# apple/ml-fastvlm

Hardware: AMD Instinct MI355X
Metric: images/sec FastViTHD encode_images @1024x1024 bf16 (higher is better)
Workload: dtype bf16; 1 GPU; BASELINE.json configs[1]: FastViTHD encoder + mlp2x_gelu projector (H=896), batch=32/GPU synthetic 1024x1024 bf16 images in [0,1), seeded synthetic weights, single GPU; global_batch=32, image_size=1024, parallelism=dp1, hip_graph=False, attention_operands=bf16, ffn_precision=auto (calibrated on the benchmark batch), range guard on

## Files before the change

ml_fastvlm_amd/csrc/ffn_fused.hip:

```cpp
#include "fvhd_common.h"
#include <stdlib.h>

typedef float f32x16 __attribute__((ext_vector_type(16)));

template <int C> __host__ __device__ __forceinline__ int w1_off(int row, int slot)
{
    if constexpr (C == 384) return row * 768 + ((slot ^ (row & 15)) << 4);
    else if constexpr (C == 192) return row * 384 + ((slot ^ ((row >> 1) & 7)) << 4);
    else return row * 192 + ((slot ^ ((row >> 2) & 3)) << 4);
}

__host__ __device__ __forceinline__ int w2_off(int row, int slot)
{
    return row * 64 + ((slot ^ ((row >> 2) & 3)) << 4);
}

struct GeluSt { f32x2 x, xc, u, q; };
#define FFN_PK(c) (f32x2{c, c})
#ifndef FVHD_FFN_GELU_DEG
#define FVHD_FFN_GELU_DEG 5
#endif
template <int H> FVHD_DEV void gelu_half(GeluSt& g, f32x2 x, f32x2& out)
{
#if FVHD_FFN_GELU_DEG == 7
    if constexpr (H == 0) {
        g.x = x;
        g.xc = f32x2{__builtin_amdgcn_fmed3f(x[0], -FVHD_GELU_CLAMP, FVHD_GELU_CLAMP), __builtin_amdgcn_fmed3f(x[1], -FVHD_GELU_CLAMP, FVHD_GELU_CLAMP)};
    } else if constexpr (H == 1) {
        g.u = g.xc * g.xc;
        g.q = __builtin_elementwise_fma(FFN_PK(FVHD_GELU_C7), g.u, FFN_PK(FVHD_GELU_C6));
    } else if constexpr (H == 2) {
        g.q = __builtin_elementwise_fma(g.q, g.u, FFN_PK(FVHD_GELU_C5));
        g.q = __builtin_elementwise_fma(g.q, g.u, FFN_PK(FVHD_GELU_C4));
    } else if constexpr (H == 3) {
        g.q = __builtin_elementwise_fma(g.q, g.u, FFN_PK(FVHD_GELU_C3));
        g.q = __builtin_elementwise_fma(g.q, g.u, FFN_PK(FVHD_GELU_C2));
    } else if constexpr (H == 4) {
        g.q = __builtin_elementwise_fma(g.q, g.u, FFN_PK(FVHD_GELU_C1));
        g.q = __builtin_elementwise_fma(g.q, g.u, FFN_PK(FVHD_GELU_C0));
    } else {
        out = g.x * __builtin_elementwise_fma(g.xc, g.q, FFN_PK(0.5f));
    }
#else
    if constexpr (H == 0) {
        g.x = x;
        g.xc = f32x2{__builtin_amdgcn_fmed3f(x[0], -FVHD_GELU5_CLAMP, FVHD_GELU5_CLAMP), __builtin_amdgcn_fmed3f(x[1], -FVHD_GELU5_CLAMP, FVHD_GELU5_CLAMP)};
    } else if constexpr (H == 1) {
        g.u = g.xc * g.xc;
        g.q = __builtin_elementwise_fma(FFN_PK(FVHD_GELU5_C5), g.u, FFN_PK(FVHD_GELU5_C4));
    } else if constexpr (H == 2) {
        g.q = __builtin_elementwise_fma(g.q, g.u, FFN_PK(FVHD_GELU5_C3));
    } else if constexpr (H == 3) {
        g.q = __builtin_elementwise_fma(g.q, g.u, FFN_PK(FVHD_GELU5_C2));
    } else if constexpr (H == 4) {
        g.q = __builtin_elementwise_fma(g.q, g.u, FFN_PK(FVHD_GELU5_C1));
        g.q = __builtin_elementwise_fma(g.q, g.u, FFN_PK(FVHD_GELU5_C0));
    } else {
        out = g.x * __builtin_elementwise_fma(g.xc, g.q, FFN_PK(0.5f));
    }
#endif
}

#ifndef FVHD_FFN_CIO384
#define FVHD_FFN_CIO384 1
#endif
#ifndef FVHD_FFN_PAIRWAIT
#define FVHD_FFN_PAIRWAIT 1
#endif
#ifndef FVHD_FFN_DMARUN
#define FVHD_FFN_DMARUN 1
#endif
#ifndef FVHD_FFN_F16
#define FVHD_FFN_F16 2
#endif
template <int C> __host__ __device__ constexpr bool ffn_f16() { return FVHD_FFN_F16 == 2 || (FVHD_FFN_F16 == 1 && C <= 192); }
typedef _Float16 f16x2 __attribute__((ext_vector_type(2)));
typedef _Float16 f16x8 __attribute__((ext_vector_type(8)));
struct GeluSt16 { f16x2 x, u, q; };
#define FFN_H2(bits) (__builtin_bit_cast(f16x2, (unsigned)(bits) * 0x10001u))
template <int K> FVHD_DEV void gelu16_stage(GeluSt16& g, f32x2 x, f16x2& out)
{
    if constexpr (K == 0) g.x = __builtin_bit_cast(f16x2, __builtin_amdgcn_cvt_pkrtz(x[0], x[1]));
    else if constexpr (K == 1) g.u = g.x * g.x;
    else if constexpr (K == 2) g.u = __builtin_elementwise_min(g.u, FFN_H2(0x3a20));
    else if constexpr (K == 3) g.q = __builtin_elementwise_fma(FFN_H2(0xc1b0), g.u, FFN_H2(0x4878));
    else if constexpr (K == 4) g.q = __builtin_elementwise_fma(g.q, g.u, FFN_H2(0xc9e5));
    else if constexpr (K == 5) g.q = __builtin_elementwise_fma(g.q, g.u, FFN_H2(0x485a));
    else if constexpr (K == 6) g.q = __builtin_elementwise_fma(g.q, g.u, FFN_H2(0xc41f));
    else if constexpr (K == 7) g.q = __builtin_elementwise_fma(g.q, g.u, FFN_H2(0x3e5f));
    else if constexpr (K == 8) asm("v_pk_fma_f16 %0, %1, %2, %3 clamp" : "=v"(g.q) : "v"(g.x), "v"(g.q), "v"(FFN_H2(0x3800)));
    else out = g.x * g.q;
}
template <int K = 0> FVHD_DEV void gelu16_dispatch(int k, GeluSt16& g, f32x2 x, f16x2& out)
{
    if constexpr (K < 10) {
        if (k == K) gelu16_stage<K>(g, x, out);
        else gelu16_dispatch<K + 1>(k, g, x, out);
    }
}

#ifdef FVHD_FFN_ABL_NOWAIT
FVHD_DEV void ffn_wait_dma() {}
#else
FVHD_DEV void ffn_wait_dma() { asm volatile("s_waitcnt vmcnt(0)" ::: "memory"); }
#endif

template <int C, int NB, int WAVES, bool DO_A, bool DO_B, bool DO_C, bool DO_DMA, int VAR, int PF, bool F16 = ffn_f16<C>(), bool BPRE = (C == 96 || F16)>
FVHD_DEV void ffn_iter(const bf16x8 (&afr)[NB][C / 16], f32x16 (&o)[NB][C / 32], f32x16 (&s_out)[NB], const f32x16 (&s_in)[NB],
                       bf16x8 (&p_out)[NB][2], const bf16x8 (&p_in)[NB][2], const char* const (&w1p)[C / 48],
                       const char* const (&w2p)[2], const int ring, const float* b1_cur, const float* b1_prev, int half,
                       const char* dma_src1, unsigned dma_dst1, bool dma1, const char* dma_src2, unsigned dma_dst2, bool dma2, int uwave)
{
    constexpr int KS = C / 16, NF = 2 * KS, NM = NF * NB;
    constexpr int NA = C / 48, CHB = 64 * C, NG = CHB / 1024;
    constexpr int UPS = 96 * NB / NM;
    constexpr int DW = WAVES, TP = 2 * NG, NPW = (TP + DW - 1) / DW;
    static_assert(TP % DW == 0, "every wave issues the same number of pieces");
    constexpr bool PIN = !(VAR & 16);
    constexpr int DSTRIDE = (VAR & 32) ? 1 : ((NM / 2) / NPW > 0 ? (NM / 2) / NPW : 1);
#define FFN_LD_W1(ks) (*(const bf16x8*)(w1p[(ks) % NA] + ring * CHB + ((ks) / NA) * NA * 32))
#define FFN_LD_W2(f) (*(const bf16x8*)(w2p[(f) & 1] + ring * CHB + ((f) >> 1) * 2048))
#define FFN_LD(f) (((f) & 1) ? FFN_LD_W2((f) >> 1) : FFN_LD_W1((f) >> 1))
#define FFN_LD_ON(f) (((f) & 1) ? DO_C : DO_A)
    bf16x8 wf[NF];
    f32x4 bv[4];
    GeluSt gs[NB][8];
    f32x2 gout[NB][8];
    GeluSt16 gs16[NB][8];
    f16x2 gout16[NB][8];
    if constexpr (DO_A && BPRE) {
#pragma unroll
        for (int q = 0; q < 4; ++q) bv[q] = *(const f32x4*)(b1_cur + 8 * q + 4 * half);
    }
    if constexpr (DO_B && !BPRE) bv[0] = *(const f32x4*)(b1_prev + 4 * half);
    constexpr bool PAIRW = FVHD_FFN_PAIRWAIT && PIN && F16 && BPRE && NB == 1 && DO_A && DO_B && DO_C && !(VAR & (4 | 8));
    constexpr int PFE = PAIRW ? 4 : PF;
#pragma unroll
    for (int f = 0; f < PFE; ++f)
        if (FFN_LD_ON(f)) wf[f] = FFN_LD(f);
    if constexpr (PIN) __builtin_amdgcn_sched_barrier(0);
#pragma unroll
    for (int m = 0; m < NM; ++m) {
        const int f = m / NB, nb = m % NB;
        if constexpr (PAIRW) {
            if ((f & 1) == 0) {
                if (f + 2 < NF) __builtin_amdgcn_s_waitcnt(0xc27f);
                else __builtin_amdgcn_s_waitcnt(0xc07f);
            }
        }
        if ((f & 1) == 0) {
            if constexpr (DO_A) {
                const int ks = f >> 1;
                if constexpr (VAR & 8) asm volatile("" ::"v"(wf[f]));
                else if (ks == 0) {
                    f32x16 z;
#pragma unroll
                    for (int r = 0; r < 16; ++r) z[r] = BPRE ? bv[r >> 2][r & 3] : 0.0f;
                    s_out[nb] = __builtin_amdgcn_mfma_f32_32x32x16_bf16(wf[f], afr[nb][ks], z, 0, 0, 0);
                } else s_out[nb] = __builtin_amdgcn_mfma_f32_32x32x16_bf16(wf[f], afr[nb][ks], s_out[nb], 0, 0, 0);
            }
        } else {
            if constexpr (DO_C) {
                const int g = f >> 1;
                if constexpr (VAR & 4) asm volatile("" ::"v"(wf[f]), "v"(p_in[nb][g & 1]));
                else if constexpr (F16)
                    o[nb][g >> 1] = __builtin_amdgcn_mfma_f32_32x32x16_f16(__builtin_bit_cast(f16x8, wf[f]), __builtin_bit_cast(f16x8, p_in[nb][g & 1]), o[nb][g >> 1], 0, 0, 0);
                else o[nb][g >> 1] = __builtin_amdgcn_mfma_f32_32x32x16_bf16(wf[f], p_in[nb][g & 1], o[nb][g >> 1], 0, 0, 0);
            }
        }
        if constexpr (PIN) __builtin_amdgcn_sched_barrier(0);
        if constexpr (PAIRW) {
            if ((f & 1) == 0) {
                if (f + 4 < NF) wf[f + 4] = FFN_LD(f + 4);
                if (f + 5 < NF) wf[f + 5] = FFN_LD(f + 5);
            }
        } else if (nb == 0 && f + PF < NF && FFN_LD_ON(f + PF)) wf[f + PF] = FFN_LD(f + PF);
        if constexpr (DO_DMA) {
#if FVHD_FFN_DMARUN
            constexpr int PPW = TP / DW, RUN = PPW % 4 == 0 ? 4 : PPW % 3 == 0 ? 3 : PPW, NRUN = PPW / RUN, RSTRIDE = (NM / 2) / NRUN > 0 ? (NM / 2) / NRUN : 1;
            static_assert(TP % DW == 0 && PPW % RUN == 0 && RUN <= 4 && DW % 2 == 0 && NG % PPW == 0, "a wave's pieces lie in one matrix");
            if (m % RSTRIDE == 0 && m / RSTRIDE < NRUN) {
                const int second = uwave >= DW / 2;
                const unsigned pc0 = (unsigned)((uwave % (DW / 2)) * PPW + (m / RSTRIDE) * RUN) * 1024u;
                const char* sb = (second ? dma_src2 : dma_src1) + pc0;
                const unsigned dst = (second ? dma_dst2 : dma_dst1) + pc0;
                if (second ? dma2 : dma1) glds16_run<RUN>(sb, (threadIdx.x & 63) * 16u, dst);
            }
#else
            if (m % DSTRIDE == 0 && m / DSTRIDE < NPW) {
                const int flat = (m / DSTRIDE) * DW + uwave;
                const int lane16 = (threadIdx.x & 63) * 16;
                const bool second = flat >= NG;
                const int pc = second ? flat - NG : flat;
                const char* src = (second ? dma_src2 : dma_src1) + pc * 1024 + lane16;
                const unsigned dst = (second ? dma_dst2 : dma_dst1) + (unsigned)pc * 1024u;
                if (second ? dma2 : dma1) glds16(src, dst);
            }
#endif
        }
        if constexpr (DO_B) {
            if constexpr (!BPRE) {
#pragma unroll
                for (int q = 1; q < 4; ++q)
                    if (m == ((24 * q * NB) / UPS >= 2 ? (24 * q * NB) / UPS - 2 : 0)) bv[q] = *(const f32x4*)(b1_prev + 8 * q + 4 * half);
            }
            if constexpr (F16) {
                constexpr int NGRP = NM / 12;
                static_assert(NGRP * UPS == 8 * NB && NGRP * 10 <= NM, "ten stages of every pair group fit into the iteration's slots");
                if (m / 10 < NGRP) {
                    const int k = m % 10;
#pragma unroll
                    for (int i = 0; i < UPS; ++i) {
                        const int pr = (m / 10) * UPS + i, gb = pr % NB, r = 2 * (pr / NB);
                        const f32x2 sv = {s_in[gb][r], s_in[gb][r + 1]};
                        if constexpr (VAR & 2) {
                            if (k == 9) gout16[gb][r >> 1] = __builtin_bit_cast(f16x2, __builtin_amdgcn_cvt_pkrtz(sv[0], sv[1]));
                        } else gelu16_dispatch(k, gs16[gb][r >> 1], sv, gout16[gb][r >> 1]);
                        if (k == 9) {
                            f16x8 pt = __builtin_bit_cast(f16x8, p_out[gb][r >> 3]);
                            pt[r & 7] = gout16[gb][r >> 1][0];
                            pt[(r & 7) + 1] = gout16[gb][r >> 1][1];
                            p_out[gb][r >> 3] = __builtin_bit_cast(bf16x8, pt);
                        }
                    }
                }
            } else
#pragma unroll
            for (int u = m * UPS / 2; u < (m + 1) * UPS / 2; ++u) {
                const int gb = u % NB, jh = u / NB, h = jh % 6, r = 2 * (jh / 6);
                f32x2 sv = {s_in[gb][r], s_in[gb][r + 1]};
                if (!BPRE && (h == 0 || ((VAR & (2 | 64)) && h == 5))) sv += f32x2{bv[r >> 2][r & 3], bv[r >> 2][(r & 3) + 1]};
                if (VAR & 2) {
                    if (h == 5) gout[gb][r >> 1] = sv;
                } else {
                    if constexpr (VAR & 64) {
                        if (h == 5) gout[gb][r >> 1] = f32x2{gelu_erf(sv[0]), gelu_erf(sv[1])};
                    } else
                    if (h == 0) gelu_half<0>(gs[gb][r >> 1], sv, gout[gb][r >> 1]);
                    else if (h == 1) gelu_half<1>(gs[gb][r >> 1], sv, gout[gb][r >> 1]);
                    else if (h == 2) gelu_half<2>(gs[gb][r >> 1], sv, gout[gb][r >> 1]);
                    else if (h == 3) gelu_half<3>(gs[gb][r >> 1], sv, gout[gb][r >> 1]);
                    else if (h == 4) gelu_half<4>(gs[gb][r >> 1], sv, gout[gb][r >> 1]);
                    else gelu_half<5>(gs[gb][r >> 1], sv, gout[gb][r >> 1]);
                }
                if (h == 5 && (r & 3) == 2) {
                    const bf16x4 pk = f32_to_bf4(f32x4{gout[gb][(r >> 1) - 1][0], gout[gb][(r >> 1) - 1][1], gout[gb][r >> 1][0], gout[gb][r >> 1][1]});
#pragma unroll
                    for (int j = 0; j < 4; ++j) p_out[gb][r >> 3][(r & 4) + j] = pk[j];
                }
            }
        }
        if constexpr (PIN) __builtin_amdgcn_sched_barrier(0);
    }
#pragma unroll
    for (int nb = 0; nb < NB; ++nb) {
        if constexpr (DO_B) asm volatile("" : "+v"(p_out[nb][0]), "+v"(p_out[nb][1]));
        if constexpr (DO_A) asm volatile("" : "+v"(s_out[nb]));
    }
#undef FFN_LD_W1
#undef FFN_LD_W2
#undef FFN_LD
#undef FFN_LD_ON
}

template <int C> FVHD_DEV int ffn_slot_of(int id)
{
    if constexpr (C == 384) return (id ^ ((id >> 4) & 15)) << 4;
    else if constexpr (C == 192) return (id ^ (((id >> 3) & 7) ^ (((id >> 6) & 1) << 3))) << 4;
    else return (id ^ ((id >> 4) & 3)) << 4;
}

template <int C, int NB, int WAVES, int VAR = 0, int PF = 3, int OCC = WAVES / 4, bool F16 = ffn_f16<C>()>
__global__ __launch_bounds__(WAVES * 64) __attribute__((amdgpu_waves_per_eu(OCC, OCC))) void ffn_fused_kernel(
    const bf16* __restrict__ A, const char* __restrict__ w1img, const char* __restrict__ w2img,
    const float* __restrict__ b1, const float* __restrict__ b2, const float* __restrict__ ls,
    bf16* X, int M, int nwg)
{
    constexpr int HID = 4 * C, KS = C / 16, NFR = C / 32, NCH = HID / 32;
    constexpr int CHB = 64 * C;
    constexpr int NG = CHB / 1024;
    static_assert(NCH % 2 == 0, "pipeline is unrolled by two");
    extern __shared__ __attribute__((aligned(16))) char smem[];
    char* w1ring = smem;
    char* w2ring = smem + 2 * CHB;
    constexpr bool CIO = C <= 192 || FVHD_FFN_CIO384;
    constexpr int STAGE0 = (C == 384 && CIO) ? 2 * CHB : 0;
    constexpr int STAGE_END = CIO ? STAGE0 + WAVES * (32 * C * 2) : 0;
    float* lb1 = (float*)(smem + (STAGE_END > 4 * CHB ? STAGE_END : 4 * CHB));

    const int tid = threadIdx.x, lane = tid & 63, wave = tid >> 6;
    const int li = lane & 31, half = lane >> 5;
    const int blk = xcd_remap(blockIdx.x, nwg);
    const int row0 = blk * (32 * NB * WAVES) + wave * (32 * NB);
    const int uwave = __builtin_amdgcn_readfirstlane(wave);
    const unsigned lds_w1 = __builtin_amdgcn_readfirstlane(lds_addr(w1ring)), lds_w2 = __builtin_amdgcn_readfirstlane(lds_addr(w2ring));

    for (int i = tid; i < HID / 4; i += WAVES * 64)
        *(f32x4*)&lb1[i * 4] = *(const f32x4*)&b1[i * 4] * (F16 ? 0.25f : 1.0f);

    const char* w1p[C / 48];
    const char* w2p[2];
#pragma unroll
    for (int k = 0; k < C / 48; ++k) w1p[k] = w1ring + w1_off<C>(li, 2 * k + half);
#pragma unroll
    for (int k = 0; k < 2; ++k) w2p[k] = w2ring + w2_off(li, 2 * k + half);

#define FFN_W1_FIRST()                                                                                                  \
    _Pragma("unroll") for (int g = 0; g < (NG + WAVES - 1) / WAVES; ++g) {                                   \
        const int piece = g * WAVES + uwave;                                                                           \
        if (NG % WAVES == 0 || piece < NG) glds16(w1img + piece * 1024 + lane * 16, lds_w1 + piece * 1024);            \
    }
    if constexpr (CIO && STAGE0 != 0) { FFN_W1_FIRST() }
    bf16x8 afr[NB][KS];
    f32x16 o[NB][NFR];
    f32x16 s0[NB], s1[NB];
    bf16x8 p0[NB][2], p1[NB][2];
    static_assert((NB == 1 || NB == 2) && WAVES % 4 == 0, "every wave transposes its tiles through its own 32-row stage, one block at a time");
    constexpr int CPR = C / 8;
    constexpr int NL = 32 * CPR / 64;
    char* stage = smem + STAGE0 + wave * (32 * C * 2);
    const size_t tile_b = (size_t)row0 * C * 2, last_b = (size_t)M * C * 2 - 16;
    constexpr size_t BLK_B = (size_t)32 * C * 2;
    if constexpr (CIO) {
        u32x4 t[NB][NL];
#pragma unroll
        for (int nb = 0; nb < NB; ++nb)
#pragma unroll
            for (int i = 0; i < NL; ++i) {
                const size_t gb = tile_b + nb * BLK_B + (size_t)(i * 64 + lane) * 16;
                t[nb][i] = *(const u32x4*)((const char*)A + (gb < last_b ? gb : last_b));
            }
#pragma unroll
        for (int nb = 0; nb < NB; ++nb) {
#pragma unroll
            for (int i = 0; i < NL; ++i) *(u32x4*)(stage + ffn_slot_of<C>(i * 64 + lane)) = t[nb][i];
#pragma unroll
            for (int ks = 0; ks < KS; ++ks) afr[nb][ks] = *(const bf16x8*)(stage + ffn_slot_of<C>(li * CPR + ks * 2 + half));
        }
    } else {
#pragma unroll
    for (int nb = 0; nb < NB; ++nb) {
        const int m_ld = min(row0 + nb * 32 + li, M - 1);
        const bf16* arow = A + (size_t)m_ld * C + half * 8;
#pragma unroll
        for (int ks = 0; ks < KS; ++ks) afr[nb][ks] = *(const bf16x8*)(arow + ks * 16);
    }
    }
    if constexpr (CIO && STAGE0 == 0) __syncthreads();
    if constexpr (!(CIO && STAGE0 != 0)) { FFN_W1_FIRST() }
#pragma unroll
    for (int nb = 0; nb < NB; ++nb) {
#pragma unroll
        for (int i = 0; i < NFR; ++i)
#pragma unroll
            for (int r = 0; r < 16; ++r) o[nb][i][r] = 0.0f;
#pragma unroll
        for (int r = 0; r < 16; ++r) { s0[nb][r] = 0.f; s1[nb][r] = 0.f; }
#pragma unroll
        for (int r = 0; r < 8; ++r) { p0[nb][0][r] = 0; p0[nb][1][r] = 0; p1[nb][0][r] = 0; p1[nb][1][r] = 0; }
    }

#define FFN_DMA_ARGS(t) w1img + (size_t)((t) < NCH ? (t) + 1 : 0) * CHB, lds_w1 + (((t) + 1) & 1) * CHB, (t) < NCH, \
                        w2img + (size_t)((t) >= 1 ? (t) - 1 : 0) * CHB, lds_w2 + (((t) + 1) & 1) * CHB, (t) >= 1, uwave
#define FFN_SYNC() ffn_wait_dma(); __syncthreads()
#define FFN_B1PREV(cur) ((cur) == lb1 ? lb1 + (NCH - 1) * 32 : (cur) - 32)
    FFN_SYNC();
    ffn_iter<C, NB, WAVES, true, false, false, !(VAR & 1), VAR, PF, F16>(afr, o, s0, s1, p1, p0, w1p, w2p, 0, lb1, FFN_B1PREV(lb1), half, FFN_DMA_ARGS(0));
    FFN_SYNC();
    ffn_iter<C, NB, WAVES, true, true, false, !(VAR & 1), VAR, PF, F16>(afr, o, s1, s0, p0, p1, w1p, w2p, 1, lb1 + 32, FFN_B1PREV(lb1 + 32), half, FFN_DMA_ARGS(1));
#pragma unroll 1
    for (int t = 2; t < NCH; t += 2) {
        FFN_SYNC();
        ffn_iter<C, NB, WAVES, true, true, true, !(VAR & 1), VAR, PF, F16>(afr, o, s0, s1, p1, p0, w1p, w2p, 0, lb1 + t * 32, FFN_B1PREV(lb1 + t * 32), half, FFN_DMA_ARGS(t));
        FFN_SYNC();
        ffn_iter<C, NB, WAVES, true, true, true, !(VAR & 1), VAR, PF, F16>(afr, o, s1, s0, p0, p1, w1p, w2p, 1, lb1 + (t + 1) * 32, FFN_B1PREV(lb1 + (t + 1) * 32), half, FFN_DMA_ARGS(t + 1));
    }
    u32x4 xq[CIO ? NB : 1][CIO ? NL : 1];
    bf16x4 xres[NB][NFR][4];
    constexpr bool XPRE = !(C == 96 && NB == 2);
#define FFN_LOAD_X()                                                                                                   \
    if constexpr (CIO) {                                                                                               \
        int xln = lane;                                                                                                \
        asm volatile("" : "+v"(xln));                                                                                  \
        _Pragma("unroll") for (int nb = 0; nb < NB; ++nb)                                                              \
            _Pragma("unroll") for (int i = 0; i < NL; ++i) {                                                           \
                const size_t gb = tile_b + nb * BLK_B + (size_t)(i * 64 + xln) * 16;                                   \
                xq[nb][i] = *(const u32x4*)((const char*)X + (gb < last_b ? gb : last_b));                             \
            }                                                                                                          \
    } else {                                                                                                           \
        _Pragma("unroll") for (int nb = 0; nb < NB; ++nb) {                                                            \
            const bf16* xrd = X + (size_t)min(row0 + nb * 32 + li, M - 1) * C + 4 * half;                              \
            _Pragma("unroll") for (int nf = 0; nf < NFR; ++nf)                                                         \
                _Pragma("unroll") for (int q = 0; q < 4; ++q) xres[nb][nf][q] = *(const bf16x4*)(xrd + nf * 32 + 8 * q); \
        }                                                                                                              \
    }
    if constexpr (XPRE) { FFN_LOAD_X() }
    FFN_SYNC();
    ffn_iter<C, NB, WAVES, false, true, true, !(VAR & 1), VAR, PF, F16>(afr, o, s0, s1, p1, p0, w1p, w2p, 0, lb1, FFN_B1PREV(lb1), half, FFN_DMA_ARGS(NCH));
    FFN_SYNC();
    ffn_iter<C, NB, WAVES, false, false, true, false, VAR, PF, F16>(afr, o, s1, s0, p0, p1, w1p, w2p, 1, lb1, FFN_B1PREV(lb1), half, FFN_DMA_ARGS(NCH));
    if constexpr (!XPRE) { FFN_LOAD_X() }
#undef FFN_LOAD_X
#undef FFN_DMA_ARGS

    if constexpr (CIO) {
    __syncthreads();
    int eln = lane;
    asm volatile("" : "+v"(eln));
    const int eli = eln & 31, ehalf = eln >> 5;
#pragma unroll
    for (int nb = 0; nb < NB; ++nb) {
#pragma unroll
    for (int i = 0; i < NL; ++i) *(u32x4*)(stage + ffn_slot_of<C>(i * 64 + eln)) = xq[nb][i];
#pragma unroll
    for (int nf = 0; nf < NFR; ++nf)
#pragma unroll
        for (int q = 0; q < 4; ++q) {
            const int n0 = nf * 32 + 8 * q + 4 * ehalf;
            char* slot = stage + ffn_slot_of<C>(eli * CPR + nf * 4 + q) + ehalf * 8;
            const f32x4 bv = *(const f32x4*)(b2 + n0), lv = *(const f32x4*)(ls + n0);
            const f32x4 rv = bf4_to_f32(*(const bf16x4*)slot);
            f32x4 v;
#pragma unroll
            for (int j = 0; j < 4; ++j) v[j] = rv[j] + lv[j] * (o[nb][nf][4 * q + j] + bv[j]);
            *(bf16x4*)slot = f32_to_bf4(v);
        }
    const int rows_ok = M - row0 - nb * 32;
#pragma unroll
    for (int i = 0; i < NL; ++i) {
        const int id = i * 64 + eln;
        const u32x4 v = *(const u32x4*)(stage + ffn_slot_of<C>(id));
        if (id < rows_ok * CPR) *(u32x4*)((char*)X + tile_b + nb * BLK_B + (size_t)id * 16) = v;
    }
    }
    } else {
#pragma unroll
    for (int nb = 0; nb < NB; ++nb) {
        const int m_row = row0 + nb * 32 + li;
        if (m_row < M) {
            bf16* xr = X + (size_t)m_row * C;
#pragma unroll
            for (int nf = 0; nf < NFR; ++nf)
#pragma unroll
                for (int q = 0; q < 4; ++q) {
                    const int n0 = nf * 32 + 8 * q + 4 * half;
                    const f32x4 bv = *(const f32x4*)(b2 + n0), lv = *(const f32x4*)(ls + n0);
                    const f32x4 rv = bf4_to_f32(xres[nb][nf][q]);
                    f32x4 v;
#pragma unroll
                    for (int j = 0; j < 4; ++j) v[j] = rv[j] + lv[j] * (o[nb][nf][4 * q + j] + bv[j]);
                    *(bf16x4*)(xr + n0) = f32_to_bf4(v);
                }
        }
    }
    }
}

#undef FFN_SYNC

#ifndef FVHD_FFN_PAIR384
#define FVHD_FFN_PAIR384 0
#endif
#if FVHD_FFN_PAIR384
template <bool DO_A, bool DO_B, bool DO_C, bool DO_DMA>
FVHD_DEV void ffn_pair_iter(const bf16x8 (&afr)[2][12], f32x16 (&o)[2][6], f32x16 (&s_out)[2], const f32x16& s_prev, bf16x8 (&p_out)[2],
                            const bf16x8 (&p_own)[2], const char* const (&w1p)[8], const char* const (&w2p)[2], const int ring,
                            const float* b1_cur, int half, const char* xs_rd, char* xs_wr, const char* px_rd, char* px_wr,
                            const char* dma_src1, unsigned dma_dst1, bool dma1, const char* dma_src2, unsigned dma_dst2, bool dma2, int uwave)
{
    constexpr int C = 384, CHB = 64 * C, NG = CHB / 1024, NFRG = 24, NM = 48, PF = 2;
#define FFP_LD(j) ((j) < 12 ? *(const bf16x8*)(w1p[(j) % 8] + ring * CHB + ((j) / 8) * 256)                                  \
                            : *(const bf16x8*)(w2p[((j) - 12) & 1] + ring * CHB + (((j) - 12) >> 1) * 2048))
#define FFP_ON(j) ((j) < 12 ? DO_A : DO_C)
    bf16x8 wf[NFRG];
    f32x4 bv[4];
    f32x4 xs[4];
    bf16x8 pp[2];
    f32x16 sf;
    GeluSt16 gs16[8];
    f16x2 gout16[8];
    if constexpr (DO_A) {
#pragma unroll
        for (int q = 0; q < 4; ++q) bv[q] = *(const f32x4*)(b1_cur + 8 * q + 4 * half);
    }
    if constexpr (DO_B) {
#pragma unroll
        for (int q = 0; q < 4; ++q) xs[q] = *(const f32x4*)(xs_rd + q * 1024);
    }
    if constexpr (DO_C) {
#pragma unroll
        for (int k = 0; k < 2; ++k) pp[k] = *(const bf16x8*)(px_rd + k * 1024);
    }
#pragma unroll
    for (int j = 0; j < PF; ++j)
        if (FFP_ON(j)) wf[j] = FFP_LD(j);
    __builtin_amdgcn_sched_barrier(0);
#pragma unroll
    for (int m = 0; m < NM; ++m) {
        const int j = m >> 1, nb = m & 1;
        if (j < 12) {
            if constexpr (DO_A) {
                if (j == 0) {
                    f32x16 z;
#pragma unroll
                    for (int r = 0; r < 16; ++r) z[r] = bv[r >> 2][r & 3];
                    s_out[nb] = __builtin_amdgcn_mfma_f32_32x32x16_bf16(wf[j], afr[nb][j], z, 0, 0, 0);
                } else s_out[nb] = __builtin_amdgcn_mfma_f32_32x32x16_bf16(wf[j], afr[nb][j], s_out[nb], 0, 0, 0);
            }
        } else {
            if constexpr (DO_C) {
                const int g = j - 12;
                const bf16x8 pb = nb == 0 ? p_own[g & 1] : pp[g & 1];
                o[nb][g >> 1] = __builtin_amdgcn_mfma_f32_32x32x16_f16(__builtin_bit_cast(f16x8, wf[j]), __builtin_bit_cast(f16x8, pb), o[nb][g >> 1], 0, 0, 0);
            }
        }
        __builtin_amdgcn_sched_barrier(0);
        if (nb == 0 && j + PF < NFRG && FFP_ON(j + PF)) wf[j + PF] = FFP_LD(j + PF);
        if constexpr (DO_DMA) {
            if (m % 8 == 0 && m / 8 < 3) {
                const int second = uwave >> 1;
                const unsigned pc0 = (unsigned)((uwave & 1) * 12 + (m / 8) * 4) * 1024u;
                const char* sb = (second ? dma_src2 : dma_src1) + pc0;
                const unsigned dst = (second ? dma_dst2 : dma_dst1) + pc0;
                if (second ? dma2 : dma1) glds16_run<4>(sb, (threadIdx.x & 63) * 16u, dst);
            }
        }
        if constexpr (DO_B) {
            if (m >= 3 && m < 7) {
#pragma unroll
                for (int i = 0; i < 4; ++i) sf[4 * (m - 3) + i] = s_prev[4 * (m - 3) + i] + xs[m - 3][i];
            }
            if (m >= 7 && m < 47) {
                const int g = (m - 7) / 10, k = (m - 7) % 10;
#pragma unroll
                for (int i = 0; i < 2; ++i) {
                    const int pr = 2 * g + i, r = 2 * pr;
                    const f32x2 sv = {sf[r], sf[r + 1]};
                    gelu16_dispatch(k, gs16[pr], sv, gout16[pr]);
// ... 117 lines not shown
        asm volatile("" : "+v"(xln));
#pragma unroll
        for (int i = 0; i < NL; ++i) {
            const size_t gb = tile_b + (size_t)(i * 64 + xln) * 16;
            xq[i] = *(const u32x4*)((const char*)X + (gb < last_b ? gb : last_b));
        }
    }
    FFP_SYNC();
    ffn_pair_iter<false, true, true, true>(afr, o, sA, sB[0], pB, pA, w1p, w2p, 0, b1base, half, FFP_X(NCH), FFP_DMA(NCH));
    FFP_SYNC();
    ffn_pair_iter<false, false, true, false>(afr, o, sB, sA[0], pA, pB, w1p, w2p, 1, b1base, half, FFP_X(NCH + 1), FFP_DMA(NCH));
#undef FFP_DMA
#undef FFP_X
#undef FFP_SYNC

    __syncthreads();
    int eln = lane;
    asm volatile("" : "+v"(eln));
    const int eli = eln & 31, ehalf = eln >> 5;
#pragma unroll
    for (int i = 0; i < NL; ++i) *(u32x4*)(stage_own + ffn_slot_of<C>(i * 64 + eln)) = xq[i];
    __syncthreads();
#pragma unroll
    for (int nb = 0; nb < 2; ++nb) {
        char* stg = nb == 0 ? stage_own : stage_par;
#pragma unroll
        for (int nf = 0; nf < 6; ++nf)
#pragma unroll
            for (int q = 0; q < 4; ++q) {
                const int n0 = (6 * role + nf) * 32 + 8 * q + 4 * ehalf;
                char* slot = stg + ffn_slot_of<C>(eli * CPR + (6 * role + nf) * 4 + q) + ehalf * 8;
                const f32x4 bv = *(const f32x4*)(b2 + n0), lv = *(const f32x4*)(ls + n0);
                const f32x4 rv = bf4_to_f32(*(const bf16x4*)slot);
                f32x4 v;
#pragma unroll
                for (int jj = 0; jj < 4; ++jj) v[jj] = rv[jj] + lv[jj] * (o[nb][nf][4 * q + jj] + bv[jj]);
                *(bf16x4*)slot = f32_to_bf4(v);
            }
    }
    __syncthreads();
    const int rows_ok = M - row_own;
#pragma unroll
    for (int i = 0; i < NL; ++i) {
        const int id = i * 64 + eln;
        const u32x4 v = *(const u32x4*)(stage_own + ffn_slot_of<C>(id));
        if (id < rows_ok * CPR) *(u32x4*)((char*)X + tile_b + (size_t)id * 16) = v;
    }
}

static hipError_t launch_ffn_pair384(hipStream_t st, const bf16* A, const char* w1img, const char* w2img, const float* b1,
                                     const float* b2, const float* ls, bf16* X, int M)
{
    const int nwg = (M + 127) / 128;
    const size_t shmem = (size_t)4 * 64 * 384 + 49152 + (size_t)4 * 384 * 4 + 128 + 256;
    static bool attr_set[64];
    int dev = 0;
    (void)hipGetDevice(&dev);
    if (!attr_set[dev & 63]) {
        hipError_t e = hipFuncSetAttribute((const void*)ffn_pair384_kernel, hipFuncAttributeMaxDynamicSharedMemorySize, (int)shmem);
        if (e != hipSuccess) return e;
        attr_set[dev & 63] = true;
    }
    hipLaunchKernelGGL(ffn_pair384_kernel, dim3(nwg), dim3(256), shmem, st, A, w1img, w2img, b1, b2, ls, X, M, nwg);
    return hipGetLastError();
}
#endif

template <typename K> static hipError_t ffn_set_lds(K kernel, size_t shmem, bool* done)
{
    int dev = 0;
    (void)hipGetDevice(&dev);
    if (done[dev & 63]) return hipSuccess;
    hipError_t e = hipFuncSetAttribute((const void*)kernel, hipFuncAttributeMaxDynamicSharedMemorySize, (int)shmem);
    if (e == hipSuccess) done[dev & 63] = true;
    return e;
}

template <int C, int NB, int WAVES, int VAR = 0, int PF = 3, int OCC = WAVES / 4, bool F16 = ffn_f16<C>()>
static hipError_t launch_ffn(hipStream_t st, const bf16* A, const char* w1img, const char* w2img, const float* b1,
                             const float* b2, const float* ls, bf16* X, int M)
{
    constexpr int ROWS = 32 * NB * WAVES;
    const int nwg = (M + ROWS - 1) / ROWS;
    const size_t rings = (size_t)4 * 64 * C, stage_end = (C == 384 ? (FVHD_FFN_CIO384 ? (size_t)2 * 64 * C : 0) : 0) + ((C <= 192 || FVHD_FFN_CIO384) ? (size_t)WAVES * 32 * C * 2 : 0);
    const size_t shmem = (stage_end > rings ? stage_end : rings) + (size_t)4 * C * 4 + 256;
    static bool attr_set[64];
    hipError_t e = ffn_set_lds(ffn_fused_kernel<C, NB, WAVES, VAR, PF, OCC, F16>, shmem, attr_set);
    if (e != hipSuccess) return e;
    hipLaunchKernelGGL((ffn_fused_kernel<C, NB, WAVES, VAR, PF, OCC, F16>), dim3(nwg), dim3(WAVES * 64), shmem, st, A, w1img, w2img, b1, b2, ls, X, M, nwg);
    return hipGetLastError();
}

extern "C" int fvhd_ffn_fused_supported(int C) { return C == 384 || C == 192 || C == 96; }

static uint16_t to_bf16(float f)
{
    uint32_t u;
    __builtin_memcpy(&u, &f, 4);
    if ((u & 0x7fffffffu) > 0x7f800000u) return (uint16_t)((u >> 16) | 0x40);
    u += 0x7fffu + ((u >> 16) & 1u);
    return (uint16_t)(u >> 16);
}

static uint16_t to_f16(float f)
{
    uint32_t u;
    __builtin_memcpy(&u, &f, 4);
    const uint16_t sign = (uint16_t)((u >> 16) & 0x8000u);
    const uint32_t a = u & 0x7fffffffu;
    if (a > 0x7f800000u) return (uint16_t)(sign | 0x7e00u);
    if (a >= 0x477ff000u) return (uint16_t)(sign | 0x7bffu);
    if (a < 0x33000001u) return sign;
    const int e = (int)(a >> 23) - 127;
    uint32_t m = (a & 0x7fffffu) | 0x800000u;
    int shift = e >= -14 ? 13 : 13 + (-14 - e);
    const uint32_t half = 1u << (shift - 1), rest = m & ((1u << shift) - 1);
    m >>= shift;
    if (rest > half || (rest == half && (m & 1u))) ++m;
    const uint32_t bits = e >= -14 ? (uint32_t)((e + 15 - 1) << 10) + m : m;
    return (uint16_t)(sign | bits);
}

extern "C" int fvhd_ffn_pack_host(int C, const float* fc1, const float* fc2, uint16_t* w1img, uint16_t* w2img, int precision)
{
    if (!fvhd_ffn_fused_supported(C) || precision < 0 || precision > 1) return 1;
    const bool f16 = precision == 0;
    const float s1 = f16 ? 0.25f : 1.0f;
    const int HID = 4 * C, NCH = HID / 32, CHE = 32 * C;
    for (int i = 0; i < (NCH + 1) * CHE; ++i) w1img[i] = 0;
    for (int ch = 0; ch < NCH; ++ch) {
        uint16_t* i1 = w1img + (size_t)ch * CHE;
        uint16_t* i2 = w2img + (size_t)ch * CHE;
        for (int row = 0; row < 32; ++row)
            for (int slot = 0; slot < C / 8; ++slot) {
                const int off = (C == 384 ? w1_off<384>(row, slot) : C == 192 ? w1_off<192>(row, slot) : w1_off<96>(row, slot)) / 2;
                for (int e = 0; e < 8; ++e) i1[off + e] = to_bf16(s1 * fc1[(size_t)(ch * 32 + row) * C + slot * 8 + e]);
            }
        for (int n = 0; n < C; ++n)
            for (int slot = 0; slot < 4; ++slot) {
                const int off = w2_off(n, slot) / 2;
                for (int e = 0; e < 8; ++e) {
                    const int pos = slot * 8 + e, kb = pos >> 4, hf = (pos >> 3) & 1, j = pos & 7;
                    const int h = 16 * kb + 8 * (j >> 2) + 4 * hf + (j & 3);
                    const float w = fc2[(size_t)n * HID + ch * 32 + h];
                    i2[off + e] = f16 ? to_f16(4.0f * w) : to_bf16(w);
                }
            }
    }
    return 0;
}

extern "C" float fvhd_ffn_half_w2_limit(void) { return 65504.0f / 4.0f; }

extern "C" int fvhd_launch_ffn_fused(hipStream_t st, const void* A, const void* w1img, const float* b1, const void* w2img,
                                     const float* b2, const float* ls, void* X, int M, int C, int precision)
{
    const bf16* a = (const bf16*)A;
    const char* w1 = (const char*)w1img;
    const char* w2 = (const char*)w2img;
    bf16* x = (bf16*)X;
    hipError_t e = hipErrorInvalidValue;
    if (M <= 0) return (int)e;
#ifdef FVHD_FFN_ABLATE
    static const int variant = [] { const char* ev = getenv("FVHD_FFN_VARIANT"); return ev ? atoi(ev) : 0; }();
#define FFN_V(CC, OCC)                                                                                                  \
    switch (variant) {                                                                                                 \
    case 1: return (int)launch_ffn<CC, 1, 4, 0, 4, OCC>(st, a, w1, w2, b1, b2, ls, x, M);                              \
// ... 55 lines not shown
```

Measured before the change: 1449 images/sec.

## Use a triple-buffered weight ring in the C=384 fused FFN kernel

For the C=384 single-block 4-wave f16 configuration, the LDS weight ring grows from two to three slots. DMA now runs two chunks ahead, and the loop is unrolled by six so ring indices stay compile-time constants. The next iteration's first four weight fragments and bias are prefetched at the end of each iteration, and __syncthreads is replaced by a bare s_barrier so the next chunk's loads can issue before the barrier. This targets the stall between barrier and first MFMA, at the cost of more LDS (which may lower occupancy), a more complex schedule, and an optional debug timestamp facility.

```diff
diff --git a/ml_fastvlm_amd/csrc/ffn_fused.hip b/ml_fastvlm_amd/csrc/ffn_fused.hip
--- a/ml_fastvlm_amd/csrc/ffn_fused.hip
+++ b/ml_fastvlm_amd/csrc/ffn_fused.hip
@@ -70,10 +70,20 @@
 #ifndef FVHD_FFN_DMARUN
 #define FVHD_FFN_DMARUN 1
 #endif
+#ifndef FVHD_FFN_RING3
+#define FVHD_FFN_RING3 1
+#endif
+#ifndef FVHD_FFN_STAMP
+#define FVHD_FFN_STAMP 0
+#endif
 #ifndef FVHD_FFN_F16
 #define FVHD_FFN_F16 2
 #endif
 template <int C> __host__ __device__ constexpr bool ffn_f16() { return FVHD_FFN_F16 == 2 || (FVHD_FFN_F16 == 1 && C <= 192); }
+template <int C, int NB, int WAVES, int VAR, bool F16> __host__ __device__ constexpr bool ffn_ring3()
+{
+    return FVHD_FFN_RING3 && FVHD_FFN_PAIRWAIT && FVHD_FFN_DMARUN && FVHD_FFN_CIO384 && C == 384 && NB == 1 && WAVES == 4 && VAR == 0 && F16;
+}
 typedef _Float16 f16x2 __attribute__((ext_vector_type(2)));
 typedef _Float16 f16x8 __attribute__((ext_vector_type(8)));
 struct GeluSt16 { f16x2 x, u, q; };
@@ -105,12 +115,35 @@
 FVHD_DEV void ffn_wait_dma() { asm volatile("s_waitcnt vmcnt(0)" ::: "memory"); }
 #endif
 
-template <int C, int NB, int WAVES, bool DO_A, bool DO_B, bool DO_C, bool DO_DMA, int VAR, int PF, bool F16 = ffn_f16<C>(), bool BPRE = (C == 96 || F16)>
+struct FfnStamps {
+#if FVHD_FFN_STAMP
+    unsigned long long v[24];
+#endif
+};
+#if FVHD_FFN_STAMP
+#ifndef FVHD_DEBUG_KNOBS
+#error "FVHD_FFN_STAMP is for the experiment library (FVHD_DEBUG_KNOBS)"
+#endif
+__device__ unsigned long long ffn_stamp_buf[8][4][16];
+#define FFN_STAMP(st, i) ((st).v[i] = __builtin_amdgcn_s_memtime())
+extern "C" int fvhd_debug_ffn_stamps(void* out, int bytes)
+{
+    if (bytes != (int)sizeof(ffn_stamp_buf)) return (int)hipErrorInvalidValue;
+    return (int)hipMemcpyFromSymbol(out, HIP_SYMBOL(ffn_stamp_buf), sizeof(ffn_stamp_buf));
+}
+#else
+#define FFN_STAMP(st, i) ((void)0)
+#endif
+
+struct FfnPre { bf16x8 wf[4]; f32x4 bv[4]; };
+template <int C, int NB, int WAVES, bool DO_A, bool DO_B, bool DO_C, bool DO_DMA, int VAR, int PF, bool F16 = ffn_f16<C>(), bool PRE_IN = false, bool PRE_OUT = false, bool BPRE = (C == 96 || F16)>
 FVHD_DEV void ffn_iter(const bf16x8 (&afr)[NB][C / 16], f32x16 (&o)[NB][C / 32], f32x16 (&s_out)[NB], const f32x16 (&s_in)[NB],
                        bf16x8 (&p_out)[NB][2], const bf16x8 (&p_in)[NB][2], const char* const (&w1p)[C / 48],
                        const char* const (&w2p)[2], const int ring, const float* b1_cur, const float* b1_prev, int half,
-                       const char* dma_src1, unsigned dma_dst1, bool dma1, const char* dma_src2, unsigned dma_dst2, bool dma2, int uwave)
-{
+                       const char* dma_src1, unsigned dma_dst1, bool dma1, const char* dma_src2, unsigned dma_dst2, bool dma2, int uwave,
+                       FfnPre& fpre, const int ring_next, const float* b1_next, FfnStamps& st, const int st0)
+{
+    FFN_STAMP(st, st0);
     constexpr int KS = C / 16, NF = 2 * KS, NM = NF * NB;
     constexpr int NA = C / 48, CHB = 64 * C, NG = CHB / 1024;
     constexpr int UPS = 96 * NB / NM;
@@ -118,9 +151,10 @@
     static_assert(TP % DW == 0, "every wave issues the same number of pieces");
     constexpr bool PIN = !(VAR & 16);
     constexpr int DSTRIDE = (VAR & 32) ? 1 : ((NM / 2) / NPW > 0 ? (NM / 2) / NPW : 1);
-#define FFN_LD_W1(ks) (*(const bf16x8*)(w1p[(ks) % NA] + ring * CHB + ((ks) / NA) * NA * 32))
-#define FFN_LD_W2(f) (*(const bf16x8*)(w2p[(f) & 1] + ring * CHB + ((f) >> 1) * 2048))
-#define FFN_LD(f) (((f) & 1) ? FFN_LD_W2((f) >> 1) : FFN_LD_W1((f) >> 1))
+#define FFN_LD_W1(ks, rg) (*(const bf16x8*)(w1p[(ks) % NA] + (rg) * CHB + ((ks) / NA) * NA * 32))
+#define FFN_LD_W2(f, rg) (*(const bf16x8*)(w2p[(f) & 1] + (rg) * CHB + ((f) >> 1) * 2048))
+#define FFN_LD_R(f, rg) (((f) & 1) ? FFN_LD_W2((f) >> 1, rg) : FFN_LD_W1((f) >> 1, rg))
+#define FFN_LD(f) FFN_LD_R(f, ring)
 #define FFN_LD_ON(f) (((f) & 1) ? DO_C : DO_A)
     bf16x8 wf[NF];
     f32x4 bv[4];
@@ -128,24 +162,35 @@
     f32x2 gout[NB][8];
     GeluSt16 gs16[NB][8];
     f16x2 gout16[NB][8];
-    if constexpr (DO_A && BPRE) {
+    if constexpr (PRE_IN) {
+#pragma unroll
+        for (int q = 0; q < 4; ++q) bv[q] = fpre.bv[q];
+    } else if constexpr (DO_A && BPRE) {
 #pragma unroll
         for (int q = 0; q < 4; ++q) bv[q] = *(const f32x4*)(b1_cur + 8 * q + 4 * half);
     }
     if constexpr (DO_B && !BPRE) bv[0] = *(const f32x4*)(b1_prev + 4 * half);
     constexpr bool PAIRW = FVHD_FFN_PAIRWAIT && PIN && F16 && BPRE && NB == 1 && DO_A && DO_B && DO_C && !(VAR & (4 | 8));
     constexpr int PFE = PAIRW ? 4 : PF;
-#pragma unroll
-    for (int f = 0; f < PFE; ++f)
-        if (FFN_LD_ON(f)) wf[f] = FFN_LD(f);
+    static_assert(!PRE_IN || PAIRW, "the carried fragments are the four of the paired form");
+    static_assert(!PRE_OUT || (PIN && NB == 1 && BPRE), "carried fragments: production form only");
+#pragma unroll
+    for (int f = 0; f < PFE; ++f) {
+        if constexpr (PRE_IN) wf[f] = fpre.wf[f];
+        else if (FFN_LD_ON(f)) wf[f] = FFN_LD(f);
+    }
     if constexpr (PIN) __builtin_amdgcn_sched_barrier(0);
 #pragma unroll
     for (int m = 0; m < NM; ++m) {
         const int f = m / NB, nb = m % NB;
         if constexpr (PAIRW) {
             if ((f & 1) == 0) {
+                if (f == 2) FFN_STAMP(st, st0 + 3);
                 if (f + 2 < NF) __builtin_amdgcn_s_waitcnt(0xc27f);
                 else __builtin_amdgcn_s_waitcnt(0xc07f);
+                if (f == 0) FFN_STAMP(st, st0 + 2);
+                if (f == 2) FFN_STAMP(st, st0 + 4);
+                if constexpr (PRE_IN || PRE_OUT) __builtin_amdgcn_sched_barrier(0);
             }
         }
         if ((f & 1) == 0) {
@@ -175,6 +220,17 @@
                 if (f + 5 < NF) wf[f + 5] = FFN_LD(f + 5);
             }
         } else if (nb == 0 && f + PF < NF && FFN_LD_ON(f + PF)) wf[f + PF] = FFN_LD(f + PF);
+        if constexpr (PRE_OUT) {
+            if (m == NM - 1) {
+#pragma unroll
+                for (int q = 0; q < 4; ++q) fpre.bv[q] = *(const f32x4*)(b1_next + 8 * q + 4 * half);
+#pragma unroll
+                for (int g = 0; g < 4; ++g) {
+                    __builtin_amdgcn_sched_barrier(0);
+                    fpre.wf[g] = FFN_LD_R(g, ring_next);
+                }
+            }
+        }
         if constexpr (DO_DMA) {
 #if FVHD_FFN_DMARUN
             constexpr int PPW = TP / DW, RUN = PPW % 4 == 0 ? 4 : PPW % 3 == 0 ? 3 : PPW, NRUN = PPW / RUN, RSTRIDE = (NM / 2) / NRUN > 0 ? (NM / 2) / NRUN : 1;
@@ -257,8 +313,10 @@
         if constexpr (DO_B) asm volatile("" : "+v"(p_out[nb][0]), "+v"(p_out[nb][1]));
         if constexpr (DO_A) asm volatile("" : "+v"(s_out[nb]));
     }
+    FFN_STAMP(st, st0 + 5);
 #undef FFN_LD_W1
 #undef FFN_LD_W2
+#undef FFN_LD_R
 #undef FFN_LD
 #undef FFN_LD_ON
 }
@@ -281,12 +339,14 @@
     constexpr int NG = CHB / 1024;
     static_assert(NCH % 2 == 0, "pipeline is unrolled by two");
     extern __shared__ __attribute__((aligned(16))) char smem[];
+    constexpr bool R3 = ffn_ring3<C, NB, WAVES, VAR, F16>();
+    constexpr int NR = R3 ? 3 : 2;
     char* w1ring = smem;
-    char* w2ring = smem + 2 * CHB;
+    char* w2ring = smem + NR * CHB;
     constexpr bool CIO = C <= 192 || FVHD_FFN_CIO384;
     constexpr int STAGE0 = (C == 384 && CIO) ? 2 * CHB : 0;
     constexpr int STAGE_END = CIO ? STAGE0 + WAVES * (32 * C * 2) : 0;
-    float* lb1 = (float*)(smem + (STAGE_END > 4 * CHB ? STAGE_END : 4 * CHB));
+    float* lb1 = (float*)(smem + (STAGE_END > 2 * NR * CHB ? STAGE_END : 2 * NR * CHB));
 
     const int tid = threadIdx.x, lane = tid & 63, wave = tid >> 6;
     const int li = lane & 31, half = lane >> 5;
@@ -304,11 +364,19 @@
     for (int k = 0; k < C / 48; ++k) w1p[k] = w1ring + w1_off<C>(li, 2 * k + half);
 #pragma unroll
     for (int k = 0; k < 2; ++k) w2p[k] = w2ring + w2_off(li, 2 * k + half);
-
+    if constexpr (R3) {
+        unsigned a1[C / 48], a2[2];
+#pragma unroll
+        for (int k = 0; k < C / 48; ++k) { a1[k] = lds_addr(w1p[k]); asm volatile("" : "+v"(a1[k])); w1p[k] = (const char*)(__attribute__((address_space(3))) char*)(size_t)a1[k]; }
+#pragma unroll
+        for (int k = 0; k < 2; ++k) { a2[k] = lds_addr(w2p[k]); asm volatile("" : "+v"(a2[k])); w2p[k] = (const char*)(__attribute__((address_space(3))) char*)(size_t)a2[k]; }
+    }
+
+    constexpr int NG0 = R3 ? 2 * NG : NG;
 #define FFN_W1_FIRST()                                                                                                  \
-    _Pragma("unroll") for (int g = 0; g < (NG + WAVES - 1) / WAVES; ++g) {                                   \
+    _Pragma("unroll") for (int g = 0; g < (NG0 + WAVES - 1) / WAVES; ++g) {                  \
         const int piece = g * WAVES + uwave;                                                                           \
-        if (NG % WAVES == 0 || piece < NG) glds16(w1img + piece * 1024 + lane * 16, lds_w1 + piece * 1024);            \
+        if (NG0 % WAVES == 0 || piece < NG0) glds16(w1img + piece * 1024 + lane * 16, lds_w1 + piece * 1024);          \
     }
     if constexpr (CIO && STAGE0 != 0) { FFN_W1_FIRST() }
     bf16x8 afr[NB][KS];
@@ -363,17 +431,51 @@
 #define FFN_DMA_ARGS(t) w1img + (size_t)((t) < NCH ? (t) + 1 : 0) * CHB, lds_w1 + (((t) + 1) & 1) * CHB, (t) < NCH, \
                         w2img + (size_t)((t) >= 1 ? (t) - 1 : 0) * CHB, lds_w2 + (((t) + 1) & 1) * CHB, (t) >= 1, uwave
 #define FFN_SYNC() ffn_wait_dma(); __syncthreads()
+#define FFN_SYNCS(s) ffn_wait_dma(); FFN_STAMP(st, (s) + 6); __syncthreads(); FFN_STAMP(st, (s) + 7)
 #define FFN_B1PREV(cur) ((cur) == lb1 ? lb1 + (NCH - 1) * 32 : (cur) - 32)
+#define FFN_DMA_ARGS3(t, r) w1img + (size_t)((t) + 2 < NCH ? (t) + 2 : NCH) * CHB, lds_w1 + (((r) + 2) % 3) * CHB, true, \
+                            w2img + (size_t)(t) * CHB, lds_w2 + (((r) + 2) % 3) * CHB, true, uwave
+#define FFN_SYNC3(s) ffn_wait_dma(); FFN_STAMP(st, (s) + 6); __builtin_amdgcn_s_barrier(); asm volatile("" ::: "memory"); FFN_STAMP(st, (s) + 7)
+    FfnPre fpre;
+    FfnStamps st;
+    if constexpr (R3) {
+        static_assert(NCH % 6 == 0 && NCH >= 12, "four steady iterations before the loop, six per trip");
+        FFN_SYNC();
+        ffn_iter<C, NB, WAVES, true, false, false, true, VAR, PF, F16>(afr, o, s0, s1, p1, p0, w1p, w2p, 0, lb1, FFN_B1PREV(lb1), half, FFN_DMA_ARGS3(0, 0), fpre, 0, lb1, st, 16);
+        FFN_SYNC3(16);
+        ffn_iter<C, NB, WAVES, true, true, false, true, VAR, PF, F16, false, true>(afr, o, s1, s0, p0, p1, w1p, w2p, 1, lb1 + 32, FFN_B1PREV(lb1 + 32), half, FFN_DMA_ARGS3(1, 1), fpre, 2, lb1 + 64, st, 16);
+        FFN_SYNC3(16);
+#define FFN_BODY_E(tt, r) ffn_iter<C, NB, WAVES, true, true, true, true, VAR, PF, F16, true, true>(afr, o, s0, s1, p1, p0, w1p, w2p, r, lb1 + (tt) * 32, FFN_B1PREV(lb1 + (tt) * 32), half, \
+                              FFN_DMA_ARGS3(tt, r), fpre, ((r) + 1) % 3, lb1 + ((tt) + 1) * 32, st, 0); FFN_SYNC3(0)
+#define FFN_BODY_O(tt, r) ffn_iter<C, NB, WAVES, true, true, true, true, VAR, PF, F16, true, true>(afr, o, s1, s0, p0, p1, w1p, w2p, r, lb1 + (tt) * 32, FFN_B1PREV(lb1 + (tt) * 32), half, \
+                              FFN_DMA_ARGS3(tt, r), fpre, ((r) + 1) % 3, lb1 + ((tt) + 1 < NCH ? (tt) + 1 : 0) * 32, st, 8); FFN_SYNC3(8)
+        FFN_BODY_E(2, 2);
+        FFN_BODY_O(3, 0);
+        FFN_BODY_E(4, 1);
+        FFN_BODY_O(5, 2);
+#pragma unroll 1
+        for (int t = 6; t < NCH; t += 6) {
+            FFN_BODY_E(t, 0);
+            FFN_BODY_O(t + 1, 1);
+            FFN_BODY_E(t + 2, 2);
+            FFN_BODY_O(t + 3, 0);
+            FFN_BODY_E(t + 4, 1);
+            FFN_BODY_O(t + 5, 2);
+        }
+#undef FFN_BODY_E
+#undef FFN_BODY_O
+    } else {
     FFN_SYNC();
-    ffn_iter<C, NB, WAVES, true, false, false, !(VAR & 1), VAR, PF, F16>(afr, o, s0, s1, p1, p0, w1p, w2p, 0, lb1, FFN_B1PREV(lb1), half, FFN_DMA_ARGS(0));
+    ffn_iter<C, NB, WAVES, true, false, false, !(VAR & 1), VAR, PF, F16>(afr, o, s0, s1, p1, p0, w1p, w2p, 0, lb1, FFN_B1PREV(lb1), half, FFN_DMA_ARGS(0), fpre, 0, lb1, st, 16);
     FFN_SYNC();
-    ffn_iter<C, NB, WAVES, true, true, false, !(VAR & 1), VAR, PF, F16>(afr, o, s1, s0, p0, p1, w1p, w2p, 1, lb1 + 32, FFN_B1PREV(lb1 + 32), half, FFN_DMA_ARGS(1));
+    ffn_iter<C, NB, WAVES, true, true, false, !(VAR & 1), VAR, PF, F16>(afr, o, s1, s0, p0, p1, w1p, w2p, 1, lb1 + 32, FFN_B1PREV(lb1 + 32), half, FFN_DMA_ARGS(1), fpre, 0, lb1, st, 16);
 #pragma unroll 1
     for (int t = 2; t < NCH; t += 2) {
-        FFN_SYNC();
-        ffn_iter<C, NB, WAVES, true, true, true, !(VAR & 1), VAR, PF, F16>(afr, o, s0, s1, p1, p0, w1p, w2p, 0, lb1 + t * 32, FFN_B1PREV(lb1 + t * 32), half, FFN_DMA_ARGS(t));
-        FFN_SYNC();
-        ffn_iter<C, NB, WAVES, true, true, true, !(VAR & 1), VAR, PF, F16>(afr, o, s1, s0, p0, p1, w1p, w2p, 1, lb1 + (t + 1) * 32, FFN_B1PREV(lb1 + (t + 1) * 32), half, FFN_DMA_ARGS(t + 1));
+        FFN_SYNCS(0);
+        ffn_iter<C, NB, WAVES, true, true, true, !(VAR & 1), VAR, PF, F16>(afr, o, s0, s1, p1, p0, w1p, w2p, 0, lb1 + t * 32, FFN_B1PREV(lb1 + t * 32), half, FFN_DMA_ARGS(t), fpre, 0, lb1, st, 0);
+        FFN_SYNCS(8);
+        ffn_iter<C, NB, WAVES, true, true, true, !(VAR & 1), VAR, PF, F16>(afr, o, s1, s0, p0, p1, w1p, w2p, 1, lb1 + (t + 1) * 32, FFN_B1PREV(lb1 + (t + 1) * 32), half, FFN_DMA_ARGS(t + 1), fpre, 0, lb1, st, 8);
+    }
     }
     u32x4 xq[CIO ? NB : 1][CIO ? NL : 1];
     bf16x4 xres[NB][NFR][4];
@@ -395,13 +497,21 @@
         }                                                                                                              \
     }
     if constexpr (XPRE) { FFN_LOAD_X() }
+    if constexpr (R3) {
+        ffn_iter<C, NB, WAVES, false, true, true, false, VAR, PF, F16>(afr, o, s0, s1, p1, p0, w1p, w2p, NCH % 3, lb1, FFN_B1PREV(lb1), half, FFN_DMA_ARGS(NCH), fpre, 0, lb1, st, 16);
+        ffn_iter<C, NB, WAVES, false, false, true, false, VAR, PF, F16>(afr, o, s1, s0, p0, p1, w1p, w2p, (NCH + 1) % 3, lb1, FFN_B1PREV(lb1), half, FFN_DMA_ARGS(NCH), fpre, 0, lb1, st, 16);
+    } else {
     FFN_SYNC();
-    ffn_iter<C, NB, WAVES, false, true, true, !(VAR & 1), VAR, PF, F16>(afr, o, s0, s1, p1, p0, w1p, w2p, 0, lb1, FFN_B1PREV(lb1), half, FFN_DMA_ARGS(NCH));
+    ffn_iter<C, NB, WAVES, false, true, true, !(VAR & 1), VAR, PF, F16>(afr, o, s0, s1, p1, p0, w1p, w2p, 0, lb1, FFN_B1PREV(lb1), half, FFN_DMA_ARGS(NCH), fpre, 0, lb1, st, 16);
     FFN_SYNC();
-    ffn_iter<C, NB, WAVES, false, false, true, false, VAR, PF, F16>(afr, o, s1, s0, p0, p1, w1p, w2p, 1, lb1, FFN_B1PREV(lb1), half, FFN_DMA_ARGS(NCH));
+    ffn_iter<C, NB, WAVES, false, false, true, false, VAR, PF, F16>(afr, o, s1, s0, p0, p1, w1p, w2p, 1, lb1, FFN_B1PREV(lb1), half, FFN_DMA_ARGS(NCH), fpre, 0, lb1, st, 16);
+    }
     if constexpr (!XPRE) { FFN_LOAD_X() }
 #undef FFN_LOAD_X
 #undef FFN_DMA_ARGS
+#undef FFN_DMA_ARGS3
+#undef FFN_SYNC3
+#undef FFN_SYNCS
 
     if constexpr (CIO) {
     __syncthreads();
@@ -454,6 +564,14 @@
         }
     }
     }
+#if FVHD_FFN_STAMP
+    if (blockIdx.x < 8 && wave < 4) {
+        unsigned long long r = 0;
+#pragma unroll
+        for (int i = 0; i < 16; ++i) r = lane == i ? st.v[i] : r;
+        if (lane < 16) ffn_stamp_buf[blockIdx.x][wave][lane] = r;
+    }
+#endif
 }
 
 #undef FFN_SYNC
@@ -737,7 +855,7 @@
 {
     constexpr int ROWS = 32 * NB * WAVES;
     const int nwg = (M + ROWS - 1) / ROWS;
-    const size_t rings = (size_t)4 * 64 * C, stage_end = (C == 384 ? (FVHD_FFN_CIO384 ? (size_t)2 * 64 * C : 0) : 0) + ((C <= 192 || FVHD_FFN_CIO384) ? (size_t)WAVES * 32 * C * 2 : 0);
+    const size_t rings = (size_t)(ffn_ring3<C, NB, WAVES, VAR, F16>() ? 6 : 4) * 64 * C, stage_end = (C == 384 ? (FVHD_FFN_CIO384 ? (size_t)2 * 64 * C : 0) : 0) + ((C <= 192 || FVHD_FFN_CIO384) ? (size_t)WAVES * 32 * C * 2 : 0);
     const size_t shmem = (stage_end > rings ? stage_end : rings) + (size_t)4 * C * 4 + 256;
     static bool attr_set[64];
     hipError_t e = ffn_set_lds(ffn_fused_kernel<C, NB, WAVES, VAR, PF, OCC, F16>, shmem, attr_set);
```

New measurement: 1460 images/sec (median of 6 runs). No clear change (+0.7%).
